# RL4M/PCRLv2

Hardware: AMD Instinct MI355X
Metric: 3D crops/sec (64x64x32, b=32) pretrain step (higher is better)
Workload: dtype bf16; 1 GPU; C2: PCRLv23d pre-train step, 64x64x32 global views x2 + 6 local 16^3, b=32/GPU, fwd+bwd+SGD; global_batch=32, parallelism=dp1

## Files before the change

### pcrlv2_amd/csrc/conv_brick.hip

```cpp
#include "internal.h"

#ifndef BRICK_ABL
#define BRICK_ABL 0
#endif
#include <mutex>

namespace {

constexpr int TD = 4, TH = 8, TW = 8;
constexpr int BRICK = TD * TH * TW;
constexpr int HH = TH + 2, HWU = TW + 2;
constexpr int HW = 16;
constexpr int HLT = 240;
template <int KD> struct BrickGeom {
  static constexpr int HD = TD + KD - 1;
  static constexpr int LINES = HD * HH;
  static constexpr int HPT = (LINES + 5) / 6;
  static constexpr int HALO_BYTES = HPT * 6 * HW * 64;
  static constexpr int TAPS = 9 * KD, NS = 3 * KD;
};

struct BrickParams {
  const bf16* x;
  const bf16* w;
  const float* bias;
  bf16* y;
  float* stats;
  int N, D, H, W;
  int K, Nc;
  int up;
  int ny;
  int sd, sh, sw, td, th, tw;
  int upc;
  const float* bias_tab;
  int cshift;
  int bd, bh, bw;
  int fsd, fsh, fsw;
  const float *aff_scale, *aff_shift;
  const bf16* res;
  float act_lo;
};

__device__ __forceinline__ int hoff_w(int row, int slot) {
  const int key = (0x78 >> (((row >> 2) & 3) * 2)) & 3;
  return row * 64 + ((slot ^ key) << 4);
}
__device__ __forceinline__ int hoff_h(int row, int slot) {
  return row * 64 + ((slot ^ (((row >> 2) & 1) << 1)) << 4);
}

template <int BN, int KD, int MODE = 0, bool AFF = false>
__global__ void __launch_bounds__(256, 2) brick_conv_kernel(const BrickParams p) {
  static_assert(!AFF || (KD == 1 && MODE == 0), "the inference epilogue exists for the 2D forward only");
  using BG = BrickGeom<KD>;
  static_assert(MODE == 0 || KD == 3, "the composed modes are 3-D");
  constexpr bool UPCF = MODE == 1, UPCD = MODE == 2;
  constexpr int HPT = BG::HPT, HALO_BYTES = BG::HALO_BYTES, NS = MODE ? 4 : BG::NS;
  constexpr int NKW = MODE ? 2 : 3;
  constexpr int FN = BN / 16;
  constexpr int WT_BYTES = 3 * BN * 64;
  extern __shared__ __attribute__((aligned(16))) char smem[];
  char* halo = smem;
  char* wbuf = smem + HALO_BYTES;

  const int tid = threadIdx.x, lane = tid & 63, wid = tid >> 6;
  const int lr = lane & 15, lg = lane >> 4;
  const int K = p.K, nchunk = K / 32;

  const int bw = p.W / TW, bh = p.H / TH, bd = p.D / TD;
  int b = blockIdx.x, ytile = blockIdx.y;
  if (p.ny > 0) {
    const int nbr = gridDim.x / p.ny;
    if ((nbr & 7) == 0) {
      const int slot = b >> 3;
      ytile = slot % p.ny;
      b = (b & 7) * (nbr >> 3) + slot / p.ny;
    } else {
      ytile = b % p.ny;
      b = b / p.ny;
    }
  } else if ((gridDim.x & 7) == 0) {
    b = (b & 7) * (gridDim.x >> 3) + (b >> 3);
  }
  const int n0 = ytile * BN;
  const int uph = UPCF ? n0 / p.upc : 0;
  const int upd = (uph >> p.bd) & 1, uphh = (uph >> p.bh) & 1, upw = (uph >> p.bw) & 1;
#define PARC(c_) ((c_) >> p.cshift)
#define PBIT(c_, b_) ((PARC(c_) >> (b_)) & 1)
#define SID(c_, s_) (MODE == 0 ? (s_) : MODE == 1 ? ((upd + ((s_) >> 1)) * 3 + uphh + ((s_)&1)) \
                                                 : ((1 - PBIT(c_, p.bd) + ((s_) >> 1)) * 3 + 1 - PBIT(c_, p.bh) + ((s_)&1)))
#define KWB(c_) (MODE == 0 ? 0 : MODE == 1 ? upw : 1 - PBIT(c_, p.bw))
  const int brick_id = b;
  const int w0 = (b % bw) * TW; b /= bw;
  const int h0 = (b % bh) * TH; b /= bh;
  const int d0 = (b % bd) * TD; b /= bd;
  const int n = b;

  const int htid = tid < HLT ? tid : tid - HLT;
  const int hq = htid % 40, hl0 = htid / 40;
  const int hslot = hq & 3;
  int grow[HPT];
  uint32_t hvalid = 0;
#pragma unroll
  for (int i = 0; i < HPT; ++i) {
    const int line = hl0 + 6 * i;
    const int hd = line / HH, hh = line % HH, hw = hq >> 2;
    const int d = d0 + hd - (KD - 1) / 2, h = h0 + hh - 1, w = w0 + hw - 1;
    const bool ok = line < BG::LINES && (unsigned)d < (unsigned)p.D && (unsigned)h < (unsigned)p.H && (unsigned)w < (unsigned)p.W;
    if (KD == 1 && p.up) {
      const int Hs = p.H >> 1, Ws = p.W >> 1;
      grow[i] = ok ? ((n * p.D + d) * Hs + (h >> 1)) * Ws + (w >> 1) : ((n * p.D + d0) * Hs + (h0 >> 1)) * Ws + (w0 >> 1);
    } else if (UPCD) {
      grow[i] = n * (8 * p.D * p.H * p.W) + (ok ? 2 * d * p.fsd + 2 * h * p.fsh + 2 * w * p.fsw : 2 * d0 * p.fsd + 2 * h0 * p.fsh + 2 * w0 * p.fsw);
    } else {
      grow[i] = n * (p.D * p.H * p.W) + (ok ? d * p.sd + h * p.sh + w * p.sw : d0 * p.sd + h0 * p.sh + w0 * p.sw);
    }
    hvalid |= (uint32_t)ok << i;
  }
  const int hdst0 = hoff_h(hl0 * HW + (hq >> 2), hslot);

  const bool wthread = BN == 64 || (tid >> 2) < BN;
  const bf16* wrow = p.w + ((int64_t)(n0 + (wthread ? (tid >> 2) : 0)) * BG::TAPS) * K + (tid & 3) * 8;
  const int wdst = hoff_w(tid >> 2, tid & 3);

  f32x4 acc[4][FN];
#pragma unroll
  for (int i = 0; i < 4; ++i)
#pragma unroll
    for (int j = 0; j < FN; ++j) acc[i][j] = f32x4{0.f, 0.f, 0.f, 0.f};

  u32x4 rh[HPT], rw[3];

#define LOAD_HALO(c_)                                                                                     \
  do {                                                                                                    \
    if (UPCD) {                                                                                           \
      const int poff = PBIT(c_, p.bd) * p.fsd + PBIT(c_, p.bh) * p.fsh + PBIT(c_, p.bw) * p.fsw;          \
      const int co0 = ((c_) - (PARC(c_) << p.cshift)) * 32 + hslot * 8;                                   \
      _Pragma("unroll") for (int i = 0; i < HPT; ++i)                                                     \
        rh[i] = *reinterpret_cast<const u32x4*>(p.x + (int64_t)(grow[i] + poff) * p.upc + co0);           \
    } else {                                                                                              \
      _Pragma("unroll") for (int i = 0; i < HPT; ++i)                                                     \
        rh[i] = *reinterpret_cast<const u32x4*>(p.x + (int64_t)grow[i] * K + (c_)*32 + hslot * 8);        \
    }                                                                                                     \
  } while (0)
#define STORE_HALO()                                                                                      \
  do {                                                                                                    \
    _Pragma("unroll") for (int i = 0; i < HPT; ++i) {                                                     \
      *reinterpret_cast<u32x4*>(halo + hdst0 + i * (6 * HW * 64)) = keep_if((hvalid >> i) & 1u, rh[i]);       \
    }                                                                                                     \
// ... 201 lines not shown
#pragma unroll
        for (int j = 0; j < FN; ++j) bv[j] = p.bias_tab[cls * p.upc + uch0 + j * 16 + lr];
      }
      char* const yrow = ybase + (int64_t)(2 * fm) * HS + (int64_t)r * WS;
#pragma unroll
      for (int j = 0; j < FN; ++j) {
        float val = acc[fm][j][r] + bv[j];
        if (AFF) {
          val = fmaf(asc[j], val, ash[j]);
          if (p.res) val += (float)*reinterpret_cast<const bf16*>(yrow + rdelta + yl + j * 32);
          val = fmaxf(val, p.act_lo);
        }
        if (!(BRICK_ABL & 1) || val == 12345.678f) *reinterpret_cast<bf16*>(yrow + yl + j * 32) = (bf16)val;
        if (!AFF) {
          s1[j] += val;
          s2[j] += val * val;
        }
      }
    }
  }
  if (!AFF && p.stats) {
    float* red = reinterpret_cast<float*>(smem);
#pragma unroll
    for (int j = 0; j < FN; ++j) {
      float a = s1[j], c2 = s2[j];
      a += __shfl_xor(a, 16, 64);
      c2 += __shfl_xor(c2, 16, 64);
      a += __shfl_xor(a, 32, 64);
      c2 += __shfl_xor(c2, 32, 64);
      if (lg == 0) {
        red[(wid * 64 + j * 16 + lr) * 2 + 0] = a;
        red[(wid * 64 + j * 16 + lr) * 2 + 1] = c2;
      }
    }
    __syncthreads();
    if (tid < BN) {
      float a = 0.f, c2 = 0.f;
#pragma unroll
      for (int q = 0; q < 4; ++q) {
        a += red[(q * 64 + tid) * 2 + 0];
        c2 += red[(q * 64 + tid) * 2 + 1];
      }
      float* o = p.stats + ((int64_t)brick_id * p.Nc + n0 + tid) * 2;
      o[0] = a;
      o[1] = c2;
    }
  }
}

}

static bool brick_natural(int D, int H, int W) { return D % TD == 0 && H % TH == 0 && W % TW == 0; }
static bool brick_permuted(int D, int H, int W) { return W % TD == 0 && D % TH == 0 && H % TW == 0; }
bool pcrl_brick_conv_eligible(int N, int D, int H, int W, int Ci, int Co, int dtype) {
  return dtype == PCRL_BF16 && (brick_natural(D, H, W) || brick_permuted(D, H, W)) && Ci % 32 == 0 && Co % 32 == 0 &&
         (int64_t)N * D * H * W < (int64_t)1 << 31;
}
int64_t pcrl_brick_conv_rows(int N, int D, int H, int W) { return (int64_t)N * D * H * W / BRICK; }

int pcrl_brick_conv_launch(const void* x, const void* wp, const float* bias, void* y, float* stats,
                           int N, int D, int H, int W, int Ci, int Co, hipStream_t stream) {
  constexpr int HB = BrickGeom<3>::HALO_BYTES;
  static std::once_flag attr_once;
  std::call_once(attr_once, [&] {
    hipFuncSetAttribute(reinterpret_cast<const void*>(brick_conv_kernel<64, 3>), hipFuncAttributeMaxDynamicSharedMemorySize, HB + 3 * 64 * 64);
    hipFuncSetAttribute(reinterpret_cast<const void*>(brick_conv_kernel<32, 3>), hipFuncAttributeMaxDynamicSharedMemorySize, HB + 3 * 32 * 64);
  });
  BrickParams p{(const bf16*)x, (const bf16*)wp, bias, (bf16*)y, stats, N, D, H, W, Ci, Co, 0, 0, H * W, W, 1, 9, 3, 1};
  if (W % TW != 0) {
    p.D = W; p.H = D; p.W = H;
    p.sd = 1; p.sh = H * W; p.sw = W;
    p.td = 1; p.th = 9; p.tw = 3;
  }
  const unsigned bricks = (unsigned)pcrl_brick_conv_rows(N, D, H, W);
  const int BN = (Co % 64 == 0 && (int64_t)bricks * (Co / 64) > 192) ? 64 : 32, ny = Co / BN;
  dim3 grid(bricks, ny);
  if (g_hooks.brick_ymap && ny > 1 && (uint64_t)bricks * ny < (1u << 31)) {
    p.ny = ny;
    grid = dim3(bricks * ny);
  }
  if (BN == 64) hipLaunchKernelGGL((brick_conv_kernel<64, 3>), grid, dim3(256), HB + 3 * 64 * 64, stream, p);
  else hipLaunchKernelGGL((brick_conv_kernel<32, 3>), grid, dim3(256), HB + 3 * 32 * 64, stream, p);
  return pcrl_check_launch("brick_conv");
}

bool pcrl_brick_conv2d_eligible(int N, int H, int W, int Ci, int Co, int dtype) {
  return dtype == PCRL_BF16 && N % TD == 0 && H % TH == 0 && W % TW == 0 && Ci % 32 == 0 && Co % 32 == 0 && (int64_t)N * H * W < (int64_t)1 << 31;
}
int64_t pcrl_brick_conv2d_rows(int N, int H, int W) { return (int64_t)(N / TD) * (H / TH) * (W / TW); }

int pcrl_brick_conv2d_launch(const void* x, const void* wp, const float* bias, void* y, float* stats, int N, int H, int W, int Ci, int Co, int up,
                             hipStream_t stream) {
  constexpr int HB = BrickGeom<1>::HALO_BYTES;
  BrickParams p{(const bf16*)x, (const bf16*)wp, bias, (bf16*)y, stats, 1, N, H, W, Ci, Co, up, 0, H * W, W, 1, 9, 3, 1};
  const unsigned bricks = (unsigned)pcrl_brick_conv2d_rows(N, H, W);
  if (Co % 64 == 0) hipLaunchKernelGGL((brick_conv_kernel<64, 1>), dim3(bricks, Co / 64), dim3(256), HB + 3 * 64 * 64, stream, p);
  else hipLaunchKernelGGL((brick_conv_kernel<32, 1>), dim3(bricks, Co / 32), dim3(256), HB + 3 * 32 * 64, stream, p);
  return pcrl_check_launch("brick_conv2d");
}

int pcrl_brick_conv2d_affine_launch(const void* x, const void* wp, const float* bias, const float* scale, const float* shift, const void* res, float act_lo,
                                    void* a, int N, int H, int W, int Ci, int Co, int up, hipStream_t stream) {
  constexpr int HB = BrickGeom<1>::HALO_BYTES;
  BrickParams p{(const bf16*)x, (const bf16*)wp, bias, (bf16*)a, nullptr, 1, N, H, W, Ci, Co, up, 0, H * W, W, 1, 9, 3, 1};
  p.aff_scale = scale; p.aff_shift = shift; p.res = (const bf16*)res; p.act_lo = act_lo;
  const unsigned bricks = (unsigned)pcrl_brick_conv2d_rows(N, H, W);
  if (Co % 64 == 0) hipLaunchKernelGGL((brick_conv_kernel<64, 1, 0, true>), dim3(bricks, Co / 64), dim3(256), HB + 3 * 64 * 64, stream, p);
  else hipLaunchKernelGGL((brick_conv_kernel<32, 1, 0, true>), dim3(bricks, Co / 32), dim3(256), HB + 3 * 32 * 64, stream, p);
  return pcrl_check_launch("brick_conv2d_affine");
}

static void upc_axes(BrickParams& p, int D, int H, int W) {
  p.sd = H * W; p.sh = W; p.sw = 1; p.td = 9; p.th = 3; p.tw = 1;
  p.bd = 2; p.bh = 1; p.bw = 0;
  p.fsd = 4 * H * W; p.fsh = 2 * W; p.fsw = 1;
  if (!brick_natural(D, H, W)) {
    p.D = W; p.H = D; p.W = H;
    p.sd = 1; p.sh = H * W; p.sw = W;
    p.td = 1; p.th = 9; p.tw = 3;
    p.bd = 0; p.bh = 2; p.bw = 1;
    p.fsd = 1; p.fsh = 4 * H * W; p.fsw = 2 * W;
  }
}
template <int BN, int MODE> static void launch_upc8(const BrickParams& p, unsigned nblocks, hipStream_t stream) {
  constexpr int HB = BrickGeom<3>::HALO_BYTES;
  static std::once_flag attr_once;
  std::call_once(attr_once, [&] {
    hipFuncSetAttribute(reinterpret_cast<const void*>(brick_conv_kernel<BN, 3, MODE>), hipFuncAttributeMaxDynamicSharedMemorySize, HB + 3 * BN * 64);
  });
  hipLaunchKernelGGL((brick_conv_kernel<BN, 3, MODE>), dim3(nblocks), dim3(256), HB + 3 * BN * 64, stream, p);
}
bool pcrl_brick8_upc_fwd_eligible(int N, int D, int H, int W, int Ci, int Co, int dtype) {
  return pcrl_brick_conv_eligible(N, D, H, W, Ci, 8 * Co, dtype) && Co % 64 == 0 && (int64_t)N * D * H * W * 8 < ((int64_t)1 << 29);
}
int pcrl_brick8_upc_fwd_launch(const void* x, const void* w3, const float* bias_tab, void* y0, float* stats, int N, int D, int H, int W, int Ci, int Co,
                               hipStream_t stream) {
  BrickParams p{(const bf16*)x, (const bf16*)w3, nullptr, (bf16*)y0, stats, N, D, H, W, Ci, 8 * Co, 0, 8 * Co / 64, 0, 0, 0, 0, 0, 0, Co, bias_tab, 0};
  upc_axes(p, D, H, W);
  const int64_t blocks = pcrl_brick_conv_rows(N, D, H, W) * p.ny;
  if (blocks >= ((int64_t)1 << 31)) return pcrl_fail(PCRL_EINVAL, "brick (composed up-conv): grid too large");
  launch_upc8<64, 1>(p, (unsigned)blocks, stream);
  return pcrl_check_launch("brick_conv (composed up-conv forward)");
}
static int upc8_cshift(int Co) {
  for (int k = 0; k < 8; ++k)
    if (Co == (32 << k)) return k;
  return -1;
}
bool pcrl_brick8_upc_dgrad_eligible(int N, int D, int H, int W, int Ci, int Co, int dtype) {
  return upc8_cshift(Co) >= 0 && pcrl_brick_conv_eligible(N, D, H, W, 8 * Co, Ci, dtype) && (int64_t)N * D * H * W * 8 < ((int64_t)1 << 29);
}
int pcrl_brick8_upc_dgrad_launch(const void* dy0, const void* wd3, void* dx, int N, int D, int H, int W, int Ci, int Co, hipStream_t stream) {
  const int64_t bricks = pcrl_brick_conv_rows(N, D, H, W);
  const int BN = (Ci % 64 == 0 && bricks * (Ci / 64) > 192) ? 64 : 32;
  BrickParams p{(const bf16*)dy0, (const bf16*)wd3, nullptr, (bf16*)dx, nullptr, N, D, H, W, 8 * Co, Ci, 0, Ci / BN, 0, 0, 0, 0, 0, 0, Co, nullptr, upc8_cshift(Co)};
  upc_axes(p, D, H, W);
  const int64_t blocks = bricks * p.ny;
  if (blocks >= ((int64_t)1 << 31)) return pcrl_fail(PCRL_EINVAL, "brick (composed up-conv data gradient): grid too large");
  if (BN == 64) launch_upc8<64, 2>(p, (unsigned)blocks, stream);
  else launch_upc8<32, 2>(p, (unsigned)blocks, stream);
  return pcrl_check_launch("brick_conv (composed up-conv data gradient)");
}
```

### pcrlv2_amd/csrc/conv_brick16.h

```cpp
#pragma once
#include "internal.h"
#include <mutex>

namespace {

constexpr int TD = 4, TH = 8, TW = 16;
constexpr int HH = TH + 2, HP = TW + 2;
template <int NW> struct B16Geom {
  static constexpr int HD = NW + 2;
  static constexpr int ROWS = HD * HH * HP;
  static constexpr int NDMA = (ROWS + 15) / 16;
  static constexpr int HALO_BYTES = NDMA * 1024;
  static constexpr int PPW = (NDMA + NW - 1) / NW;
};
constexpr int NS = 9;


struct Brick16Params {
  const bf16* x;
  const bf16* w;
  const float* bias;
  bf16* y;
  float* stats;
  int N, D, H, W;
  int K, Nc;
  int ny;
  int upc;
  const float* bias_tab;
  int cshift;
  const bf16* bn_y;
  const float *bn_scale, *bn_shift, *bn_mean, *bn_rstd;
  float act_lo;
};

__device__ __forceinline__ int key_w(int hw) { return ((0xFC30 >> hw) & 1) << 1; }
__device__ __forceinline__ int woff(int row, int slot) {
  const int key = (0x78 >> (((row >> 2) & 3) * 2)) & 3;
  return row * 64 + ((slot ^ key) << 4);
}

__device__ __forceinline__ void lds_dma16_masked(uint64_t base, uint32_t voff, uint32_t& okmask, uint32_t& chain, uint32_t lds_dst, uint64_t exec_all) {
  uint32_t t;
  asm volatile("v_and_b32 %0, 1, %1\n\tv_cmpx_ne_u32_e32 0, %0\n\ts_mov_b32 m0, %4\n\ts_nop 0\n\tglobal_load_lds_dwordx4 %3, %5\n\ts_mov_b64 exec, %6"
               : "=&v"(t), "+v"(okmask), "+v"(chain)
               : "v"(voff), "s"(lds_dst), "s"(base), "s"(exec_all)
               : "memory", "vcc");
}

template <int BN, int MODE = 0, int PERM = 0, int NW = 4, bool BNR = false, bool INF = false>
__global__ void __launch_bounds__(NW * 64, NW == 4 ? 2 : 1) brick16_conv_kernel(const Brick16Params p) {
  static_assert(!INF || ((MODE == 0 || MODE == 3) && NW == 4 && !BNR), "the inference epilogue exists for the plain 4-plane forward only (3D, and the 2D path's 3x3 form)");
  static_assert(!BNR || ((MODE == 0 || MODE == 3) && NW == 4), "the BatchNorm-reduce epilogue exists for the plain 4-plane data gradient only (3D, and the 2D path's 3x3 form)");
  using G = B16Geom<NW>;
  constexpr int ROWS = G::ROWS, NDMA = G::NDMA, HALO_BYTES = G::HALO_BYTES, HD = G::HD;
  constexpr int FN = BN / 16;
  constexpr bool UPCF = MODE == 1, UPCD = MODE == 2, P2D = MODE == 3;
  constexpr int NSK = P2D ? 3 : (MODE ? 4 : NS);
  constexpr int TAPS = P2D ? 9 : 27;
  extern __shared__ __attribute__((aligned(16))) char smem[];
  char* halo = smem;
  char* wbuf = smem + HALO_BYTES;

  const int tid = threadIdx.x, lane = tid & 63, wid = __builtin_amdgcn_readfirstlane(tid >> 6);
  const int lr = lane & 15, lg = lane >> 4;
  const int K = p.K, nchunk = K / 32;

  const int bw = p.W / TW, bh = p.H / TH, bd = p.D / NW;
  int b = blockIdx.x, ytile = blockIdx.y;
  if (p.ny > 0) {
    const int nbr = gridDim.x / p.ny;
    if ((nbr & 7) == 0) {
      const int slot = b >> 3;
      ytile = slot % p.ny;
      b = (b & 7) * (nbr >> 3) + slot / p.ny;
    } else {
      ytile = b % p.ny;
      b = b / p.ny;
    }
  } else if ((gridDim.x & 7) == 0) {
    b = (b & 7) * (gridDim.x >> 3) + (b >> 3);
  }
  const int n0 = ytile * BN;
#define BITD(x_) (((x_) >> 2) & 1)
#define BITH(x_) (PERM ? ((x_)&1) : (((x_) >> 1) & 1))
#define BITW(x_) (PERM ? (((x_) >> 1) & 1) : ((x_)&1))
#define VOX(n_, d_, h_, w_) (PERM ? (((int64_t)(n_)*p.D + (d_)) * p.W + (w_)) * p.H + (h_) : (((int64_t)(n_)*p.D + (d_)) * p.H + (h_)) * p.W + (w_))
#define FVOX(n_, d_, h_, w_) (PERM ? (((int64_t)(n_) * (2 * p.D) + (d_)) * (2 * p.W) + (w_)) * (2 * p.H) + (h_) \
                                   : (((int64_t)(n_) * (2 * p.D) + (d_)) * (2 * p.H) + (h_)) * (2 * p.W) + (w_))
#define WTAP(s9_, j_) ((PERM ? ((s9_) / 3) * 9 + (j_)*3 + (s9_) % 3 : (s9_)*3 + (j_)) - (MODE == 3 ? 9 : 0))
  const int uph = UPCF ? n0 / p.upc : 0, ukd0 = BITD(uph), ukh0 = BITH(uph);
#define PARC(c_) ((c_) >> p.cshift)
#define SID(c_, s_) (MODE == 0 ? (s_) : MODE == 3 ? 3 + (s_) : MODE == 1 ? ((ukd0 + ((s_) >> 1)) * 3 + ukh0 + ((s_)&1)) \
                                                 : ((1 - BITD(PARC(c_)) + ((s_) >> 1)) * 3 + 1 - BITH(PARC(c_)) + ((s_)&1)))
#define KWB(c_) (MODE == 0 || MODE == 3 ? 0 : MODE == 1 ? BITW(uph) : 1 - BITW(PARC(c_)))
  const int brick_lin = b;
  const int w0 = (b % bw) * TW; b /= bw;
  const int h0 = (b % bh) * TH; b /= bh;
  const int d0 = (b % bd) * NW; b /= bd;
  const int n = b;

  constexpr int PPW = G::PPW;
  constexpr int RSTEP = 16 * NW, QL = RSTEP / HP;
  static_assert(PPW <= 17 && RSTEP - QL * HP < HP, "plan masks hold 16 steps; at most one line wrap per step");
  const uint32_t lds_base = (uint32_t)(uintptr_t)(__attribute__((address_space(3))) char*)smem;
  int RS, LS, PS;
  if (UPCD) {
    const int v2 = 4 * p.upc;
    RS = PERM ? v2 * (2 * p.H) : v2;
    LS = PERM ? v2 : v2 * (2 * p.W);
    PS = v2 * (2 * p.H) * (2 * p.W);
  } else {
    RS = PERM ? 2 * K * p.H : 2 * K;
    LS = PERM ? 2 * K : 2 * K * p.W;
    PS = 2 * K * p.H * p.W;
  }
  const int C1 = QL * LS + (RSTEP - QL * HP) * RS, C2 = LS - HP * RS, C3 = PS - HH * LS;
#define CHUNK_OFS(c_) (UPCD ? (uint32_t)(((BITD(PARC(c_)) * (2 * p.H) * (2 * p.W) + (PERM ? BITW(PARC(c_)) * (2 * p.H) + BITH(PARC(c_)) \
                                                                                       : BITH(PARC(c_)) * (2 * p.W) + BITW(PARC(c_)))) * p.upc \
                                          + ((c_) - (PARC(c_) << p.cshift)) * 32) * 2)                                               \
                            : (uint32_t)(c_) * 64u)
  const uint64_t hbase = (uint64_t)(uintptr_t)p.x + (UPCD ? (uint64_t)(FVOX(n, 2 * (d0 - 1), 2 * (h0 - 1), 2 * (w0 - 1)) * (int64_t)(2 * p.upc))
                                                        : (uint64_t)(VOX(n, d0 - 1, h0 - 1, w0 - 1) * (int64_t)(2 * K)));
  uint32_t hoff0 = 0, m_step = 0, m_ko = 0;
  {
    int prevL = 0, prevP = 0, key0 = 0;
#pragma unroll
    for (int i = 0; i < PPW; ++i) {
      const int piece = wid + NW * i, row = piece * 16 + (lane >> 2);
      const int L = row / HP, hw = row - L * HP, P = L / HH, hh = L - P * HH;
      const int d = d0 + P - 1, h = h0 + hh - 1, w = w0 + hw - 1;
      const bool inside = row < ROWS && (unsigned)d < (unsigned)p.D && (unsigned)h < (unsigned)p.H && (unsigned)w < (unsigned)p.W;
      const bool used = P2D ? (P != 0 && P != HD - 1)
                            : (!UPCF || (P != (ukd0 ? 0 : HD - 1) && hh != (ukh0 ? 0 : HH - 1) && hw != (BITW(uph) ? 0 : HP - 1)));
      const bool ok = inside && used;
      const int key = key_w(hw) >> 1;
      if (i == 0) {
        hoff0 = (uint32_t)(P * PS + hh * LS + hw * RS + (((lane & 3) ^ (key << 1)) << 4)) | (ok ? 1u : 0u);
        key0 = key;
      } else {
        m_step |= (uint32_t)(L - prevL - QL) << (i - 1);
        m_step |= (uint32_t)(P - prevP) << (15 + i);
        m_ko |= (ok ? 1u : 0u) << (i - 1);
        m_ko |= (uint32_t)(key ^ key0) << (15 + i);
      }
      prevL = L;
      prevP = P;
      if (!inside && row < ROWS) *reinterpret_cast<u32x4*>(halo + piece * 1024 + lane * 16) = u32x4{0u, 0u, 0u, 0u};
    }
  }
  uint2* plan_lds = reinterpret_cast<uint2*>(smem + (NW == 4 ? ROWS * 64 : HALO_BYTES + 3 * BN * 64)) + wid * 16 + (lane >> 2);
  *plan_lds = uint2{m_step, m_ko};
  asm volatile("" : "+v"(hoff0));
// ... 332 lines not shown
          const float yv = (float)*reinterpret_cast<const bf16*>(ytile + (fm * 16 + r) * (BN * 2) + jx * 32);
          const float dz = bsc[j] * yv + bsh[j] > 0.f ? acc[fm][j][r] : 0.f;
          s1[j] += dz;
          s2[j] += dz * (yv - bmu[j]) * brs[j];
        }
      asm volatile("" : "+v"(s1[j]), "+v"(s2[j])::"memory");
    }
  }
  if (p.stats) {
    float* red = reinterpret_cast<float*>(smem);
#pragma unroll
    for (int j = 0; j < FN; ++j) {
      float a = s1[j], c2 = s2[j];
      a += __shfl_xor(a, 16, 64);
      c2 += __shfl_xor(c2, 16, 64);
      a += __shfl_xor(a, 32, 64);
      c2 += __shfl_xor(c2, 32, 64);
      if (lg == 0) {
        red[(wid * 64 + j * 16 + lr) * 2 + 0] = a;
        red[(wid * 64 + j * 16 + lr) * 2 + 1] = c2;
      }
    }
    __syncthreads();
    const int half = tid >> 6, ch = tid & 63;
    if (half < NW / 4 && ch < BN) {
      float a = 0.f, c2 = 0.f;
#pragma unroll
      for (int q = 0; q < 4; ++q) {
        a += red[((half * 4 + q) * 64 + ch) * 2 + 0];
        c2 += red[((half * 4 + q) * 64 + ch) * 2 + 1];
      }
      const int64_t brick_id = NW == 4 ? (int64_t)brick_lin : (((int64_t)n * (p.D / 4) + (d0 >> 2) + half) * bh + h0 / TH) * bw + w0 / TW;
      float* o = p.stats + (brick_id * p.Nc + n0 + ch) * 2;
      o[0] = a;
      o[1] = c2;
    }
  }
}

#undef BITD
#undef BITH
#undef BITW
#undef VOX
#undef FVOX

inline int brick16_perm(int D, int H, int W) {
  if (D % TD == 0 && H % TH == 0 && W % TW == 0) return 1;
  if (D % TD == 0 && W % TH == 0 && H % TW == 0) return 2;
  return 0;
}


template <int BN, int MODE, int NW = 4, bool BNR = false, bool INF = false>
inline int launch16(Brick16Params p, dim3 grid, hipStream_t stream, const char* what) {
  constexpr size_t lds = B16Geom<NW>::HALO_BYTES + 3 * BN * 64 + (NW == 4 ? 0 : 1024);
  static std::once_flag attr_once;
  std::call_once(attr_once, [&] {
    (void)hipFuncSetAttribute(reinterpret_cast<const void*>(brick16_conv_kernel<BN, MODE, 0, NW, BNR, INF>), hipFuncAttributeMaxDynamicSharedMemorySize, lds);
    (void)hipFuncSetAttribute(reinterpret_cast<const void*>(brick16_conv_kernel<BN, MODE, 1, NW, BNR, INF>), hipFuncAttributeMaxDynamicSharedMemorySize, lds);
  });
  if (brick16_perm(p.D, p.H, p.W) == 2) {
    std::swap(p.H, p.W);
    hipLaunchKernelGGL((brick16_conv_kernel<BN, MODE, 1, NW, BNR, INF>), grid, dim3(NW * 64), lds, stream, p);
  } else {
    hipLaunchKernelGGL((brick16_conv_kernel<BN, MODE, 0, NW, BNR, INF>), grid, dim3(NW * 64), lds, stream, p);
  }
  return pcrl_check_launch(what);
}


}
```

### pcrlv2_amd/csrc/conv_brick16.hip

```cpp
#include "conv_brick16.h"

bool pcrl_brick16_conv_eligible(int N, int D, int H, int W, int Ci, int Co, int dtype) {
  return g_hooks.brick16_on && dtype == PCRL_BF16 && brick16_perm(D, H, W) != 0 && Ci % 32 == 0 && Co % 32 == 0 && (int64_t)N * D * H * W < ((int64_t)1 << 29) &&
         (int64_t)20 * Ci * H * W < ((int64_t)1 << 31) && (int64_t)54 * Ci * Co < ((int64_t)1 << 32);
}
int64_t pcrl_brick16_conv_rows(int N, int D, int H, int W) { return (int64_t)N * D * H * W / (TD * TH * TW); }

int pcrl_brick16_conv_launch(const void* x, const void* wp, const float* bias, void* y, float* stats,
                             int N, int D, int H, int W, int Ci, int Co, hipStream_t stream) {
  Brick16Params p{(const bf16*)x, (const bf16*)wp, bias, (bf16*)y, stats, N, D, H, W, Ci, Co, 0, 0, nullptr, 0};
  const int BN = Co % 64 == 0 ? 64 : 32, ny = Co / BN;
  const int planes = g_hooks.brick16_planes, nw8_mode = planes >= 0 ? planes : 0;
  int64_t bricks = pcrl_brick16_conv_rows(N, D, H, W);
  const bool nw8 = nw8_mode > 0 && BN == 64 && D % 8 == 0 && (nw8_mode == 2 || (ny >= 2 && (bricks / 2) * ny >= 256));
  if (nw8) bricks /= 2;
  if (bricks * ny >= ((int64_t)1 << 31)) return pcrl_fail(PCRL_EINVAL, "brick16_conv: grid too large");
  dim3 grid((unsigned)bricks, ny);
  if (ny > 1) {
    p.ny = ny;
    grid = dim3((unsigned)(bricks * ny));
  }
  if (nw8) return launch16<64, 0, 8>(p, grid, stream, "brick16_conv (8 planes)");
  return BN == 64 ? launch16<64, 0>(p, grid, stream, "brick16_conv") : launch16<32, 0>(p, grid, stream, "brick16_conv");
}


bool pcrl_brick16_conv2d_eligible(int N, int H, int W, int Ci, int Co, int dtype) {
  return g_hooks.brick16_on && dtype == PCRL_BF16 && N % TD == 0 && brick16_perm(N, H, W) != 0 && Ci % 32 == 0 && Co % 32 == 0 &&
         (int64_t)N * H * W < ((int64_t)1 << 29) && (int64_t)20 * Ci * H * W < ((int64_t)1 << 31) && (int64_t)18 * Ci * Co < ((int64_t)1 << 32);
}
int64_t pcrl_brick16_conv2d_rows(int N, int H, int W) { return (int64_t)N * H * W / (TD * TH * TW); }
int pcrl_brick16_conv2d_launch(const void* x, const void* wp, const float* bias, void* y, float* stats, int N, int H, int W, int Ci, int Co, hipStream_t stream) {
  Brick16Params p{(const bf16*)x, (const bf16*)wp, bias, (bf16*)y, stats, 1, N, H, W, Ci, Co, 0, 0, nullptr, 0};
  const int BN = Co % 64 == 0 ? 64 : 32, ny = Co / BN;
  const int64_t bricks = pcrl_brick16_conv2d_rows(N, H, W);
  if (bricks * ny >= ((int64_t)1 << 31)) return pcrl_fail(PCRL_EINVAL, "brick16_conv2d: grid too large");
  dim3 grid((unsigned)bricks, ny);
  if (ny > 1) {
    p.ny = ny;
    grid = dim3((unsigned)(bricks * ny));
  }
  return BN == 64 ? launch16<64, 3>(p, grid, stream, "brick16_conv2d") : launch16<32, 3>(p, grid, stream, "brick16_conv2d");
}
```

### pcrlv2_amd/csrc/conv_to1_brick.hip

```cpp
#include "internal.h"
#include <mutex>

namespace {

constexpr int TD = 4, TH = 8, TW = 8;
constexpr int HD = TD + 2, HH = TH + 2, HWU = TW + 2;
constexpr int ZROWS = HD * HH * HWU;
constexpr int NFRAG = (ZROWS + 15) / 16;
constexpr int HROWS = NFRAG * 16;
constexpr int HALO_BYTES = HROWS * 64;
constexpr int HPT = (HROWS * 4 + 255) / 256;
constexpr int FPW = (NFRAG + 3) / 4;
constexpr int ZA = 17, ZB = 13;
#ifndef TO1_ZT
#define TO1_ZT 1
#endif
constexpr int ZP = 612;
constexpr int Z_BYTES = TO1_ZT ? 16 * ZP * 4 : ZROWS * ZA * 4;

struct To1Params {
  const bf16* x;
  const float* w_ref;
  const bf16* w_img;
  const float* bias;
  float* y;
  float* stats;
  int N, D, H, W, C;
};

__device__ __forceinline__ int hoff_w(int row, int slot) {
  const int key = (0x78 >> (((row >> 2) & 3) * 2)) & 3;
  return row * 64 + ((slot ^ key) << 4);
}
__device__ __forceinline__ int hoff_h(int row, int slot) { return row * 64 + ((slot ^ (((row >> 2) & 1) << 1)) << 4); }

__global__ void __launch_bounds__(256) to1_pack_kernel(const float* __restrict__ w_ref, bf16* __restrict__ img, int C) {
  const int idx = blockIdx.x * 256 + threadIdx.x;
  if (idx >= C * 32) return;
  const int c = idx >> 5, t = idx & 31;
  const float v = t < 27 ? w_ref[c * 27 + t] : 0.f;
  const int chunk = c >> 5, k = c & 31;
  *reinterpret_cast<bf16*>(reinterpret_cast<char*>(img) + chunk * 2048 + hoff_w(t, k >> 3) + (k & 7) * 2) = (bf16)v;
}

__global__ void __launch_bounds__(256, 3) to1_brick_fwd_kernel(const To1Params p) {
  extern __shared__ __attribute__((aligned(16))) char smem[];
  char* halo = smem;
  const int C = p.C, nchunk = C / 32;
  char* wl = smem + HALO_BYTES;
  const int tid = threadIdx.x, lane = tid & 63, wid = tid >> 6;
  const int lr = lane & 15, lg = lane >> 4;

  const int bw = p.W / TW, bh = p.H / TH, bd = p.D / TD;
  int b = blockIdx.x;
  if ((gridDim.x & 7) == 0) b = (b & 7) * (gridDim.x >> 3) + (b >> 3);
  const int brick_id = b;
  const int w0 = (b % bw) * TW; b /= bw;
  const int h0 = (b % bh) * TH; b /= bh;
  const int d0 = (b % bd) * TD; b /= bd;
  const int n = b;

  if (p.w_img) {
    for (int i = tid; i < nchunk * 128; i += 256)
      *reinterpret_cast<u32x4*>(wl + i * 16) = *reinterpret_cast<const u32x4*>(reinterpret_cast<const char*>(p.w_img) + i * 16);
  } else {
    for (int idx = tid; idx < C * 32; idx += 256) {
      const int c = idx >> 5, t = idx & 31;
      const float v = t < 27 ? p.w_ref[c * 27 + t] : 0.f;
      const int chunk = c >> 5, k = c & 31;
      *reinterpret_cast<bf16*>(wl + chunk * 2048 + hoff_w(t, k >> 3) + (k & 7) * 2) = (bf16)v;
    }
  }

  int grow[HPT];
  uint32_t hvalid = 0;
#pragma unroll
  for (int i = 0; i < HPT; ++i) {
    const int row = (tid + 256 * i) >> 2;
    const int hd = row / (HH * HWU), rem = row % (HH * HWU), hh = rem / HWU, hw = rem % HWU;
    const int d = d0 + hd - 1, h = h0 + hh - 1, w = w0 + hw - 1;
    const bool ok = row < ZROWS && (unsigned)d < (unsigned)p.D && (unsigned)h < (unsigned)p.H && (unsigned)w < (unsigned)p.W;
    grow[i] = ok ? ((n * p.D + d) * p.H + h) * p.W + w : ((n * p.D + d0) * p.H + h0) * p.W + w0;
    hvalid |= (uint32_t)ok << i;
  }
  const int hslot = tid & 3;
  u32x4 rh[HPT];
#define T1_LOAD_HALO(c_)                                                                                  \
  do {                                                                                                    \
    _Pragma("unroll") for (int i = 0; i < HPT; ++i)                                                       \
      rh[i] = *reinterpret_cast<const u32x4*>(p.x + (int64_t)grow[i] * C + (c_)*32 + hslot * 8);          \
  } while (0)
#define T1_STORE_HALO()                                                                                   \
  do {                                                                                                    \
    _Pragma("unroll") for (int i = 0; i < HPT; ++i)                                                       \
      if (tid + 256 * i < HROWS * 4)                                                                      \
        *reinterpret_cast<u32x4*>(halo + hoff_h((tid + 256 * i) >> 2, hslot)) = keep_if((hvalid >> i) & 1u, rh[i]); \
  } while (0)

  f32x4 acc[FPW][2];
#pragma unroll
  for (int f = 0; f < FPW; ++f)
#pragma unroll
    for (int j = 0; j < 2; ++j) acc[f][j] = f32x4{0.f, 0.f, 0.f, 0.f};
  const int aoff = hoff_h(wid * 16 + lr, lg);
  const int boff = hoff_w(lr, lg);

  T1_LOAD_HALO(0);
  T1_STORE_HALO();
  __syncthreads();
  for (int c = 0; c < nchunk; ++c) {
    if (c + 1 < nchunk) T1_LOAD_HALO(c + 1);
    const char* wt = wl + c * 2048;
    const bf16x8 fb0 = *reinterpret_cast<const bf16x8*>(wt + boff);
// ... 58 lines not shown
  for (int f = 0; f < FPW; ++f)
#pragma unroll
    for (int r = 0; r < 4; ++r) {
      const int row = (wid + 4 * f) * 16 + 4 * lg + r;
      if (row < ZROWS && lr < 11) zl[row * ZB + lr] = acc[f][1][r];
    }
  __syncthreads();
#pragma unroll
  for (int t = 16; t < 27; ++t) {
    const int kd = t / 9, kh = (t / 3) % 3, kw = t % 3;
    out += zl[(vrow + (kd * HH + kh) * HWU + kw) * ZB + (t - 16)];
  }
#endif
  p.y[(((int64_t)n * p.D + d0 + vd) * p.H + h0 + vh) * p.W + w0 + vw] = out;
  if (p.stats) {
    __shared__ float red[8];
    const float s1 = wave_sum(out), s2 = wave_sum(out * out);
    if (lane == 0) {
      red[wid * 2 + 0] = s1;
      red[wid * 2 + 1] = s2;
    }
    __syncthreads();
    if (tid == 0) {
      p.stats[(int64_t)brick_id * 2 + 0] = (red[0] + red[2]) + (red[4] + red[6]);
      p.stats[(int64_t)brick_id * 2 + 1] = (red[1] + red[3]) + (red[5] + red[7]);
    }
  }
}

}

bool pcrl_to1_brick_eligible(int N, int D, int H, int W, int C, int taps, int dtype) {
  return dtype == PCRL_BF16 && taps == 27 && D % TD == 0 && H % TH == 0 && W % TW == 0 && C % 32 == 0 && C <= 512 &&
         (int64_t)N * D * H * W < (int64_t)1 << 31;
}
int64_t pcrl_to1_brick_rows(int N, int D, int H, int W) { return (int64_t)N * (D / TD) * (H / TH) * (W / TW); }

static size_t to1_brick_ws_bytes(int C) { return (size_t)(C / 32) * 2048; }

int pcrl_to1_brick_launch(const void* x, const float* w_ref, const float* bias, float* y, float* stats, void* ws, size_t ws_bytes, int N, int D, int H,
                          int W, int C, hipStream_t stream) {
  const int lds_w = HALO_BYTES + (C / 32) * 2048;
  const int lds = lds_w > Z_BYTES ? lds_w : Z_BYTES;
  static std::once_flag attr_once;
  std::call_once(attr_once, [&] {
    (void)hipFuncSetAttribute(reinterpret_cast<const void*>(to1_brick_fwd_kernel), hipFuncAttributeMaxDynamicSharedMemorySize, HALO_BYTES + 16 * 2048);
  });
  const bf16* img = nullptr;
  if (ws && ws_bytes >= to1_brick_ws_bytes(C)) {
    img = (const bf16*)ws;
    hipLaunchKernelGGL(to1_pack_kernel, dim3((unsigned)((C * 32 + 255) / 256)), dim3(256), 0, stream, w_ref, (bf16*)ws, C);
    if (int e = pcrl_check_launch("to1_pack")) return e;
  }
  To1Params p{(const bf16*)x, w_ref, img, bias, y, stats, N, D, H, W, C};
  hipLaunchKernelGGL(to1_brick_fwd_kernel, dim3((unsigned)pcrl_to1_brick_rows(N, D, H, W)), dim3(256), lds, stream, p);
  return pcrl_check_launch("to1_brick_fwd");
}
```

### pcrlv2_amd/csrc/core.hip

```cpp
#include "internal.h"

static thread_local char g_err[512] = "";

int pcrl_fail(int code, const char* fmt, ...) {
  va_list ap;
  va_start(ap, fmt);
  vsnprintf(g_err, sizeof(g_err), fmt, ap);
  va_end(ap);
  return code;
}

int pcrl_check_launch(const char* what) {
  hipError_t e = hipGetLastError();
  if (e != hipSuccess) return pcrl_fail(PCRL_ELAUNCH, "%s: launch failed: %s", what, hipGetErrorString(e));
  return PCRL_OK;
}

extern "C" const char* pcrl_version(void) { return "pcrl_hip 0.1 (gfx950)"; }
extern "C" const char* pcrl_last_error(void) { return g_err; }

extern "C" int pcrl_zero(void* p, size_t bytes, pcrl_stream_t stream) {
  PCRL_REQUIRE(p && bytes > 0, "zero: bad arguments");
  const hipError_t e = hipMemsetAsync(p, 0, bytes, as_stream(stream));
  if (e != hipSuccess) return pcrl_fail(PCRL_ELAUNCH, "zero: hipMemsetAsync failed: %s", hipGetErrorString(e));
  return PCRL_OK;
}

PcrlHooks g_hooks;

extern "C" void pcrl_debug_set_conv_impl(int impl) {
  g_hooks.conv_impl = (impl >= 3 && impl <= 6) ? 0 : impl;
  g_hooks.brick_ymap = impl != 3;
  g_hooks.brick16_on = impl == 0 || impl == 5 || impl == 6;
  g_hooks.brick16_planes = impl == 5 ? 0 : impl == 6 ? 2 : -1;
}
extern "C" void pcrl_debug_set_wgrad_impl(int impl) {
  g_hooks.wgrad_impl = impl == 1 ? 1 : 0;
  g_hooks.wb_xcd = impl == 0 || impl == 4 || impl == 6;
  g_hooks.wb_order = impl == 0 || impl == 5 || impl == 6;
  g_hooks.wb_tiles = impl != 6;
}
extern "C" void pcrl_debug_set_wgrad_tr(int on) { g_hooks.wgrad_tr = on; }
extern "C" void pcrl_debug_set_conv2d_impl(int impl) { g_hooks.conv2d_impl = impl; }
extern "C" void pcrl_debug_set_reduce_repeat(int n) { g_hooks.reduce_repeat = n < 1 ? 1 : n; }

const PcrlEnv& pcrl_env() {
  static const PcrlEnv env = [] {
    const char *b = getenv("PCRL_DGRAD_BNRED"), *v = getenv("PCRL_IGEMM_VMAJOR"), *t = getenv("PCRL_UPC_PACK_TILED");
    return PcrlEnv{b && b[0] == '0', v ? atoi(v) == 1 ? 8 : atoi(v) : 8, !(t && t[0] == '0')};
  }();
  return env;
}
```

### pcrlv2_amd/csrc/internal.h

```cpp
#pragma once
#include "common.h"
#include <atomic>

struct PcrlHooks {
  std::atomic<int> conv_impl{0};
  std::atomic<int> brick_ymap{1};
  std::atomic<int> brick16_on{1};
  std::atomic<int> brick16_planes{-1};
  std::atomic<int> wgrad_impl{0};
  std::atomic<int> wgrad_tr{1};
  std::atomic<int> wb_xcd{1};
  std::atomic<int> wb_order{1};
  std::atomic<int> wb_tiles{1};
  std::atomic<int> conv2d_impl{0};
  std::atomic<int> reduce_repeat{1};
};
extern PcrlHooks g_hooks;

struct PcrlEnv {
  bool dgrad_bnred_off;
  int igemm_vmajor_max;
  bool upc_pack_tiled;
};
const PcrlEnv& pcrl_env();

bool pcrl_brick_conv_eligible(int N, int D, int H, int W, int Ci, int Co, int dtype);
int64_t pcrl_brick_conv_rows(int N, int D, int H, int W);
int pcrl_brick_conv_launch(const void* x, const void* wp, const float* bias, void* y, float* stats, int N, int D, int H, int W, int Ci, int Co, hipStream_t stream);
bool pcrl_brick_conv2d_eligible(int N, int H, int W, int Ci, int Co, int dtype);
int64_t pcrl_brick_conv2d_rows(int N, int H, int W);
int pcrl_brick_conv2d_launch(const void* x, const void* wp, const float* bias, void* y, float* stats, int N, int H, int W, int Ci, int Co, int up, hipStream_t stream);
int pcrl_brick_conv2d_affine_launch(const void* x, const void* wp, const float* bias, const float* scale, const float* shift, const void* res, float act_lo,
                                    void* a, int N, int H, int W, int Ci, int Co, int up, hipStream_t stream);
bool pcrl_brick8_upc_fwd_eligible(int N, int D, int H, int W, int Ci, int Co, int dtype);
int pcrl_brick8_upc_fwd_launch(const void* x, const void* w3, const float* bias_tab, void* y0, float* stats, int N, int D, int H, int W, int Ci, int Co, hipStream_t stream);
bool pcrl_brick8_upc_dgrad_eligible(int N, int D, int H, int W, int Ci, int Co, int dtype);
int pcrl_brick8_upc_dgrad_launch(const void* dy0, const void* wd3, void* dx, int N, int D, int H, int W, int Ci, int Co, hipStream_t stream);

bool pcrl_brick16_conv_eligible(int N, int D, int H, int W, int Ci, int Co, int dtype);
int64_t pcrl_brick16_conv_rows(int N, int D, int H, int W);
int pcrl_brick16_conv_launch(const void* x, const void* wp, const float* bias, void* y, float* stats, int N, int D, int H, int W, int Ci, int Co, hipStream_t stream);
bool pcrl_brick16_conv2d_eligible(int N, int H, int W, int Ci, int Co, int dtype);
int64_t pcrl_brick16_conv2d_rows(int N, int H, int W);
int pcrl_brick16_conv2d_launch(const void* x, const void* wp, const float* bias, void* y, float* stats, int N, int H, int W, int Ci, int Co, hipStream_t stream);

bool pcrl_brick16_upc_fwd_eligible(int N, int D, int H, int W, int Ci, int Co, int dtype);
int pcrl_brick16_upc_fwd_launch(const void* x, const void* w3, const float* bias_tab, void* y0, float* stats, int N, int D, int H, int W, int Ci, int Co, hipStream_t stream);
bool pcrl_brick16_upc_dgrad_eligible(int N, int D, int H, int W, int Ci, int Co, int dtype);
int pcrl_brick16_upc_dgrad_launch(const void* dy0, const void* wd3, void* dx, int N, int D, int H, int W, int Ci, int Co, hipStream_t stream);

int pcrl_brick16_conv_affine_launch(const void* x, const void* wp, const float* bias, const float* scale, const float* shift, float act_lo, void* a,
                                    int N, int D, int H, int W, int Ci, int Co, hipStream_t stream);
int pcrl_brick16_conv2d_affine_launch(const void* x, const void* wp, const float* bias, const float* scale, const float* shift, float act_lo, void* a,
                                      int N, int H, int W, int Ci, int Co, hipStream_t stream);

int pcrl_brick16_dgrad_bnred_launch(const void* dy, const void* wp, void* dx, const void* bn_y, const float* scale, const float* shift, const float* mean,
                                    const float* rstd, float* partial, int N, int D, int H, int W, int Ci, int Co, hipStream_t stream);
int pcrl_brick16_dgrad2d_bnred_launch(const void* dy, const void* wp, void* dx, const void* bn_y, const float* scale, const float* shift, const float* mean,
                                      const float* rstd, float* partial, int N, int H, int W, int Ci, int Co, hipStream_t stream);

bool pcrl_convt_up2_eligible(int Ci, int Co, int dtype);
int pcrl_convt_up2_launch(const void* x, const void* wp, const float* bias, void* y, int N, int D, int H, int W, int Ci, int Co, hipStream_t stream);

int pcrl_upc_fwd_launch(const void* x, const void* wf, const float* bias_tab, void* y0, float* stats, int N, int D, int H, int W, int Ci, int Co, int dtype, hipStream_t stream);
int64_t pcrl_upc_dgrad_ws_bytes(int N, int D, int H, int W, int Ci, int Co);
int pcrl_upc_dgrad_launch(const void* dy0, const void* wd, void* dx, void* ws, int64_t ws_bytes, int N, int D, int H, int W, int Ci, int Co, int dtype, hipStream_t stream);
int pcrl_gemm_planes_launch(const void* a, const void* b, float* z, int64_t M, int K, int Nc, int dtype, hipStream_t stream);
int pcrl_pointwise_planes_launch(const void* x, const void* wt, float* z, int64_t M, int C, int dtype, hipStream_t stream);

bool pcrl_to1_brick_eligible(int N, int D, int H, int W, int C, int taps, int dtype);
// ... 106 lines not shown
```

Baseline: 1094 crops/s.

## Walk conv bricks in cache-friendly clusters instead of raster order

Adds a configurable brick traversal that maps block indices to spatial bricks in compact clusters. Cluster shape is chosen to minimise the cut surface, within a cap of concurrent blocks. It applies to the 3D/2D brick conv, brick16 and to1 kernels, so neighbouring blocks share halo rows in L2 and duplicate fetches drop. The cost is extra integer division in the block-index decode, plus a new debug hook that can restore the old walk.

```diff
diff --git a/pcrlv2_amd/csrc/conv_brick.hip b/pcrlv2_amd/csrc/conv_brick.hip
--- a/pcrlv2_amd/csrc/conv_brick.hip
+++ b/pcrlv2_amd/csrc/conv_brick.hip
@@ -39,6 +39,7 @@
   const float *aff_scale, *aff_shift;
   const bf16* res;
   float act_lo;
+  BrickWalk walk;
 };
 
 __device__ __forceinline__ int hoff_w(int row, int slot) {
@@ -90,11 +91,9 @@
 #define SID(c_, s_) (MODE == 0 ? (s_) : MODE == 1 ? ((upd + ((s_) >> 1)) * 3 + uphh + ((s_)&1)) \
                                                  : ((1 - PBIT(c_, p.bd) + ((s_) >> 1)) * 3 + 1 - PBIT(c_, p.bh) + ((s_)&1)))
 #define KWB(c_) (MODE == 0 ? 0 : MODE == 1 ? upw : 1 - PBIT(c_, p.bw))
-  const int brick_id = b;
-  const int w0 = (b % bw) * TW; b /= bw;
-  const int h0 = (b % bh) * TH; b /= bh;
-  const int d0 = (b % bd) * TD; b /= bd;
-  const int n = b;
+  const BrickPos bp = pcrl_brick_walk(b, bw, bh, bd, p.walk);
+  const int brick_id = pcrl_brick_canon(bp, bw, bh, bd);
+  const int w0 = bp.w * TW, h0 = bp.h * TH, d0 = bp.d * TD, n = bp.n;
 
   const int htid = tid < HLT ? tid : tid - HLT;
   const int hq = htid % 40, hl0 = htid / 40;
@@ -402,6 +401,7 @@
 
 static bool brick_natural(int D, int H, int W) { return D % TD == 0 && H % TH == 0 && W % TW == 0; }
 static bool brick_permuted(int D, int H, int W) { return W % TD == 0 && D % TH == 0 && H % TW == 0; }
+static void brick_set_walk(BrickParams& p, bool flat = false) { p.walk = pcrl_brick_walk_for(p.W / TW, p.H / TH, p.D / TD, TW, TH, TD, 64, flat); }
 bool pcrl_brick_conv_eligible(int N, int D, int H, int W, int Ci, int Co, int dtype) {
   return dtype == PCRL_BF16 && (brick_natural(D, H, W) || brick_permuted(D, H, W)) && Ci % 32 == 0 && Co % 32 == 0 &&
          (int64_t)N * D * H * W < (int64_t)1 << 31;
@@ -422,6 +422,7 @@
     p.sd = 1; p.sh = H * W; p.sw = W;
     p.td = 1; p.th = 9; p.tw = 3;
   }
+  brick_set_walk(p);
   const unsigned bricks = (unsigned)pcrl_brick_conv_rows(N, D, H, W);
   const int BN = (Co % 64 == 0 && (int64_t)bricks * (Co / 64) > 192) ? 64 : 32, ny = Co / BN;
   dim3 grid(bricks, ny);
@@ -443,6 +444,7 @@
                              hipStream_t stream) {
   constexpr int HB = BrickGeom<1>::HALO_BYTES;
   BrickParams p{(const bf16*)x, (const bf16*)wp, bias, (bf16*)y, stats, 1, N, H, W, Ci, Co, up, 0, H * W, W, 1, 9, 3, 1};
+  brick_set_walk(p, true);
   const unsigned bricks = (unsigned)pcrl_brick_conv2d_rows(N, H, W);
   if (Co % 64 == 0) hipLaunchKernelGGL((brick_conv_kernel<64, 1>), dim3(bricks, Co / 64), dim3(256), HB + 3 * 64 * 64, stream, p);
   else hipLaunchKernelGGL((brick_conv_kernel<32, 1>), dim3(bricks, Co / 32), dim3(256), HB + 3 * 32 * 64, stream, p);
@@ -454,6 +456,7 @@
   constexpr int HB = BrickGeom<1>::HALO_BYTES;
   BrickParams p{(const bf16*)x, (const bf16*)wp, bias, (bf16*)a, nullptr, 1, N, H, W, Ci, Co, up, 0, H * W, W, 1, 9, 3, 1};
   p.aff_scale = scale; p.aff_shift = shift; p.res = (const bf16*)res; p.act_lo = act_lo;
+  brick_set_walk(p, true);
   const unsigned bricks = (unsigned)pcrl_brick_conv2d_rows(N, H, W);
   if (Co % 64 == 0) hipLaunchKernelGGL((brick_conv_kernel<64, 1, 0, true>), dim3(bricks, Co / 64), dim3(256), HB + 3 * 64 * 64, stream, p);
   else hipLaunchKernelGGL((brick_conv_kernel<32, 1, 0, true>), dim3(bricks, Co / 32), dim3(256), HB + 3 * 32 * 64, stream, p);
@@ -471,6 +474,7 @@
     p.bd = 0; p.bh = 2; p.bw = 1;
     p.fsd = 1; p.fsh = 4 * H * W; p.fsw = 2 * W;
   }
+  brick_set_walk(p);
 }
 template <int BN, int MODE> static void launch_upc8(const BrickParams& p, unsigned nblocks, hipStream_t stream) {
   constexpr int HB = BrickGeom<3>::HALO_BYTES;
diff --git a/pcrlv2_amd/csrc/conv_brick16.h b/pcrlv2_amd/csrc/conv_brick16.h
--- a/pcrlv2_amd/csrc/conv_brick16.h
+++ b/pcrlv2_amd/csrc/conv_brick16.h
@@ -31,6 +31,7 @@
   const bf16* bn_y;
   const float *bn_scale, *bn_shift, *bn_mean, *bn_rstd;
   float act_lo;
+  BrickWalk walk;
 };
 
 __device__ __forceinline__ int key_w(int hw) { return ((0xFC30 >> hw) & 1) << 1; }
@@ -93,11 +94,11 @@
 #define SID(c_, s_) (MODE == 0 ? (s_) : MODE == 3 ? 3 + (s_) : MODE == 1 ? ((ukd0 + ((s_) >> 1)) * 3 + ukh0 + ((s_)&1)) \
                                                  : ((1 - BITD(PARC(c_)) + ((s_) >> 1)) * 3 + 1 - BITH(PARC(c_)) + ((s_)&1)))
 #define KWB(c_) (MODE == 0 || MODE == 3 ? 0 : MODE == 1 ? BITW(uph) : 1 - BITW(PARC(c_)))
-  const int brick_lin = b;
-  const int w0 = (b % bw) * TW; b /= bw;
-  const int h0 = (b % bh) * TH; b /= bh;
-  const int d0 = (b % bd) * NW; b /= bd;
-  const int n = b;
+  const BrickPos bp = pcrl_brick_walk(b, bw, bh, bd, p.walk);
+  const int brick_lin = pcrl_brick_canon(bp, bw, bh, bd);
+#define B16_PIN(v_) (NW == 8 ? __builtin_amdgcn_readfirstlane(v_) : (v_))
+  const int w0 = B16_PIN(bp.w * TW), h0 = B16_PIN(bp.h * TH), d0 = B16_PIN(bp.d * NW), n = B16_PIN(bp.n);
+#undef B16_PIN
 
   constexpr int PPW = G::PPW;
   constexpr int RSTEP = 16 * NW, QL = RSTEP / HP;
@@ -536,15 +537,18 @@
 
 
 template <int BN, int MODE, int NW = 4, bool BNR = false, bool INF = false>
-inline int launch16(Brick16Params p, dim3 grid, hipStream_t stream, const char* what) {
+inline int launch16(Brick16Params p, dim3 grid, hipStream_t stream, const char* what, bool keep_old_walk = false) {
   constexpr size_t lds = B16Geom<NW>::HALO_BYTES + 3 * BN * 64 + (NW == 4 ? 0 : 1024);
   static std::once_flag attr_once;
   std::call_once(attr_once, [&] {
     (void)hipFuncSetAttribute(reinterpret_cast<const void*>(brick16_conv_kernel<BN, MODE, 0, NW, BNR, INF>), hipFuncAttributeMaxDynamicSharedMemorySize, lds);
     (void)hipFuncSetAttribute(reinterpret_cast<const void*>(brick16_conv_kernel<BN, MODE, 1, NW, BNR, INF>), hipFuncAttributeMaxDynamicSharedMemorySize, lds);
   });
-  if (brick16_perm(p.D, p.H, p.W) == 2) {
-    std::swap(p.H, p.W);
+  const bool perm = brick16_perm(p.D, p.H, p.W) == 2;
+  if (perm) std::swap(p.H, p.W);
+  p.walk = pcrl_brick_walk_for(p.W / TW, p.H / TH, p.D / NW, TW, TH, NW, NW == 4 ? 64 : 32, MODE == 3);
+  if (keep_old_walk && g_hooks.brick_walk == 1) p.walk = BrickWalk{p.W / TW, p.H / TH, p.D / NW};
+  if (perm) {
     hipLaunchKernelGGL((brick16_conv_kernel<BN, MODE, 1, NW, BNR, INF>), grid, dim3(NW * 64), lds, stream, p);
   } else {
     hipLaunchKernelGGL((brick16_conv_kernel<BN, MODE, 0, NW, BNR, INF>), grid, dim3(NW * 64), lds, stream, p);
diff --git a/pcrlv2_amd/csrc/conv_brick16.hip b/pcrlv2_amd/csrc/conv_brick16.hip
--- a/pcrlv2_amd/csrc/conv_brick16.hip
+++ b/pcrlv2_amd/csrc/conv_brick16.hip
@@ -21,7 +21,8 @@
     grid = dim3((unsigned)(bricks * ny));
   }
   if (nw8) return launch16<64, 0, 8>(p, grid, stream, "brick16_conv (8 planes)");
-  return BN == 64 ? launch16<64, 0>(p, grid, stream, "brick16_conv") : launch16<32, 0>(p, grid, stream, "brick16_conv");
+  const int plane = brick16_perm(D, H, W) == 2 ? (H / TW) * (W / TH) : (W / TW) * (H / TH);
+  return BN == 64 ? launch16<64, 0>(p, grid, stream, "brick16_conv") : launch16<32, 0>(p, grid, stream, "brick16_conv", 2 * plane <= 64);
 }
 
 
diff --git a/pcrlv2_amd/csrc/conv_to1_brick.hip b/pcrlv2_amd/csrc/conv_to1_brick.hip
--- a/pcrlv2_amd/csrc/conv_to1_brick.hip
+++ b/pcrlv2_amd/csrc/conv_to1_brick.hip
@@ -26,6 +26,7 @@
   float* y;
   float* stats;
   int N, D, H, W, C;
+  BrickWalk walk;
 };
 
 __device__ __forceinline__ int hoff_w(int row, int slot) {
@@ -54,11 +55,9 @@
   const int bw = p.W / TW, bh = p.H / TH, bd = p.D / TD;
   int b = blockIdx.x;
   if ((gridDim.x & 7) == 0) b = (b & 7) * (gridDim.x >> 3) + (b >> 3);
-  const int brick_id = b;
-  const int w0 = (b % bw) * TW; b /= bw;
-  const int h0 = (b % bh) * TH; b /= bh;
-  const int d0 = (b % bd) * TD; b /= bd;
-  const int n = b;
+  const BrickPos bp = pcrl_brick_walk(b, bw, bh, bd, p.walk);
+  const int brick_id = pcrl_brick_canon(bp, bw, bh, bd);
+  const int w0 = bp.w * TW, h0 = bp.h * TH, d0 = bp.d * TD, n = bp.n;
 
   if (p.w_img) {
     for (int i = tid; i < nchunk * 128; i += 256)
@@ -223,7 +222,7 @@
     hipLaunchKernelGGL(to1_pack_kernel, dim3((unsigned)((C * 32 + 255) / 256)), dim3(256), 0, stream, w_ref, (bf16*)ws, C);
     if (int e = pcrl_check_launch("to1_pack")) return e;
   }
-  To1Params p{(const bf16*)x, w_ref, img, bias, y, stats, N, D, H, W, C};
+  To1Params p{(const bf16*)x, w_ref, img, bias, y, stats, N, D, H, W, C, pcrl_brick_walk_for(W / TW, H / TH, D / TD, TW, TH, TD, 64)};
   hipLaunchKernelGGL(to1_brick_fwd_kernel, dim3((unsigned)pcrl_to1_brick_rows(N, D, H, W)), dim3(256), lds, stream, p);
   return pcrl_check_launch("to1_brick_fwd");
 }
diff --git a/pcrlv2_amd/csrc/core.hip b/pcrlv2_amd/csrc/core.hip
--- a/pcrlv2_amd/csrc/core.hip
+++ b/pcrlv2_amd/csrc/core.hip
@@ -29,10 +29,20 @@
 PcrlHooks g_hooks;
 
 extern "C" void pcrl_debug_set_conv_impl(int impl) {
-  g_hooks.conv_impl = (impl >= 3 && impl <= 6) ? 0 : impl;
+  g_hooks.conv_impl = (impl >= 3 && impl <= 8) ? 0 : impl;
   g_hooks.brick_ymap = impl != 3;
-  g_hooks.brick16_on = impl == 0 || impl == 5 || impl == 6;
+  g_hooks.brick16_on = impl == 0 || (impl >= 5 && impl <= 8);
   g_hooks.brick16_planes = impl == 5 ? 0 : impl == 6 ? 2 : -1;
+  g_hooks.brick_walk = impl == 7 ? 0 : impl == 8 ? 2 : 1;
+}
+extern "C" void pcrl_debug_brick_walk_decode(int pos, int bw, int bh, int bd, int cw, int ch, int cd, int* out) {
+  const BrickPos b = pcrl_brick_walk(pos, bw, bh, bd, BrickWalk{cw, ch, cd});
+  out[0] = b.n; out[1] = b.d; out[2] = b.h; out[3] = b.w;
+  out[4] = pcrl_brick_canon(b, bw, bh, bd);
+}
+extern "C" void pcrl_debug_brick_walk_shape(int bw, int bh, int bd, int tw, int th, int td, int cap, int flat, int* out) {
+  const BrickWalk k = pcrl_brick_walk_shape(bw, bh, bd, tw, th, td, cap, flat != 0, true);
+  out[0] = k.cw; out[1] = k.ch; out[2] = k.cd;
 }
 extern "C" void pcrl_debug_set_wgrad_impl(int impl) {
   g_hooks.wgrad_impl = impl == 1 ? 1 : 0;
diff --git a/pcrlv2_amd/csrc/internal.h b/pcrlv2_amd/csrc/internal.h
--- a/pcrlv2_amd/csrc/internal.h
+++ b/pcrlv2_amd/csrc/internal.h
@@ -14,8 +14,59 @@
   std::atomic<int> wb_tiles{1};
   std::atomic<int> conv2d_impl{0};
   std::atomic<int> reduce_repeat{1};
+  std::atomic<int> brick_walk{1};
 };
 extern PcrlHooks g_hooks;
+
+struct BrickWalk {
+  int cw, ch, cd;
+};
+struct BrickPos {
+  int n, d, h, w;
+};
+__host__ __device__ inline BrickPos pcrl_brick_walk(int pos, int bw, int bh, int bd, const BrickWalk k) {
+  const int per = bw * bh * bd;
+  const int n = pos / per;
+  int r = pos - n * per;
+  const int sd = k.cd * bh * bw, kd = r / sd;
+  r -= kd * sd;
+  const int dl = bd - kd * k.cd < k.cd ? bd - kd * k.cd : k.cd;
+  const int sh = k.ch * dl * bw, kh = r / sh;
+  r -= kh * sh;
+  const int hl = bh - kh * k.ch < k.ch ? bh - kh * k.ch : k.ch;
+  const int sw = k.cw * dl * hl, kw = r / sw;
+  r -= kw * sw;
+  const int wl = bw - kw * k.cw < k.cw ? bw - kw * k.cw : k.cw;
+  const int d = r / (hl * wl);
+  r -= d * (hl * wl);
+  const int h = r / wl;
+  return BrickPos{n, kd * k.cd + d, kh * k.ch + h, kw * k.cw + r - h * wl};
+}
+__host__ __device__ inline int pcrl_brick_canon(const BrickPos& b, int bw, int bh, int bd) { return ((b.n * bd + b.d) * bh + b.h) * bw + b.w; }
+inline BrickWalk pcrl_brick_walk_shape(int bw, int bh, int bd, int tw, int th, int td, int cap, bool flat, bool clustered) {
+  if (!clustered) return BrickWalk{bw, bh, bd};
+  BrickWalk best{1, 1, 1};
+  const int64_t ed = (int64_t)bd * td, eh = (int64_t)bh * th, ew = (int64_t)bw * tw;
+  int64_t bcost = -1;
+  for (int cd = 1; cd <= (flat ? 1 : bd) && cd <= cap; ++cd)
+    for (int ch = 1; ch <= bh && cd * ch <= cap; ++ch)
+      for (int cw = 1; cw <= bw && cd * ch * cw <= cap; ++cw) {
+        const int64_t nd = (bd + cd - 1) / cd, nh = (bh + ch - 1) / ch, nw = (bw + cw - 1) / cw;
+        const int64_t cost = (flat ? 0 : nd * eh * ew) + nh * ed * ew + nw * ed * eh;
+        if (bcost < 0 || cost < bcost) {
+          best = BrickWalk{cw, ch, cd};
+          bcost = cost;
+        }
+      }
+  return best;
+}
+inline BrickWalk pcrl_brick_walk_for(int bw, int bh, int bd, int tw, int th, int td, int cap, bool flat = false) {
+  const int mode = g_hooks.brick_walk;
+  if (mode == 2) return BrickWalk{1, bh < 2 ? bh : 2, flat || bd < 2 ? 1 : 2};
+  return pcrl_brick_walk_shape(bw, bh, bd, tw, th, td, cap, flat, mode != 0);
+}
+extern "C" void pcrl_debug_brick_walk_decode(int pos, int bw, int bh, int bd, int cw, int ch, int cd, int* out);
+extern "C" void pcrl_debug_brick_walk_shape(int bw, int bh, int bd, int tw, int th, int td, int cap, int flat, int* out);
 
 struct PcrlEnv {
   bool dgrad_bnred_off;
```

Measured after the change: 1093 crops/s (median of 2 runs). Within noise of the previous version (-0.0%).
